# musheen/LevelSetFortran

Measured on AMD Instinct MI355X. Metric: cell-updates/s (WENO5 reinit, 512^3 fp64), higher is better.
Workload: dtype f64

## Files before the change

levelsetfortran_amd/csrc/lsf_cell.hpp:

```cpp
#pragma once
#include <hip/hip_runtime.h>

namespace lsf {

__device__ __forceinline__ double fmax2(double a, double b) { return (a > b) ? a : b; }
__device__ __forceinline__ double fmin2(double a, double b) { return (a < b) ? a : b; }
__device__ __forceinline__ double smax(double a, double b) { return __builtin_fmax(a, b); }
__device__ __forceinline__ double smin(double a, double b) { return __builtin_fmin(a, b); }

__device__ __forceinline__ double recip_refined(double d)
{
    double r = __builtin_amdgcn_rcp(d);
    double e = __builtin_fma(-d, r, 1.0);
    r = __builtin_fma(r, e, r);
    e = __builtin_fma(-d, r, 1.0);
    return __builtin_fma(r, e, r);
}
__device__ __forceinline__ double div_by(double n, double d, double r)
{
#pragma clang fp contract(off)
    const double q = n * r;
    const double e = __builtin_fma(-d, q, n);
    return __builtin_fma(e, r, q);
}
// ... 154 lines not shown
{
    double r = __builtin_amdgcn_rcp(x);
    const double e = __builtin_fma(-x, r, 1.0);
    return __builtin_fma(r, e, r);
}

__device__ __forceinline__ void weno_axis_fast(const double q[7], double floor2, bool yquirk, double& dm,
                                               double& dp)
{
    const double d0 = q[1] - q[0], d1 = q[2] - q[1], d2 = q[3] - q[2];
    const double d3 = q[4] - q[3], d4 = q[5] - q[4], d5 = q[6] - q[5];
    const double am = d1 - d0, bm = d2 - d1, cp = d3 - d2, bp = d4 - d3, ap = d5 - d4;
    const double e_ab = ap - bp, e_bc = bp - cp, e_cm = cp - bm, e_mm = am - bm;
    const double t0p = __builtin_fma(-3.0, bp, ap), t1p = bp + cp, t2p = __builtin_fma(3.0, cp, -bm);
    const double t0m = __builtin_fma(-3.0, bm, am), t1m = bm + cp, t2m = __builtin_fma(3.0, cp, -bp);

    const double mid = __builtin_fmax(__builtin_fmax(__builtin_fabs(d1), __builtin_fabs(d2)),
                                      __builtin_fmax(__builtin_fabs(d3), __builtin_fabs(d4)));
    const double mp = yquirk ? mid : __builtin_fmax(mid, __builtin_fabs(d5));
    const double mm = __builtin_fmax(mid, __builtin_fabs(d0));
    constexpr double C = 13.0 / 3.0;
    const double fl = C * floor2;
    const double epsp = __builtin_fma((1.E-6 / 3.0) * mp, mp, fl);
    const double epsm = __builtin_fma((1.E-6 / 3.0) * mm, mm, fl);

    const double c_ab = C * e_ab, c_bc = C * e_bc, c_cm = C * e_cm, c_mm = C * e_mm;
    const double q0p = __builtin_fma(t0p, t0p, __builtin_fma(c_ab, e_ab, epsp));
    const double q1p = __builtin_fma(t1p, t1p, __builtin_fma(c_bc, e_bc, epsp));
    const double q2p = __builtin_fma(t2p, t2p, __builtin_fma(c_cm, e_cm, epsp));
    const double q0m = __builtin_fma(t0m, t0m, __builtin_fma(c_mm, e_mm, epsm));
    const double q1m = __builtin_fma(t1m, t1m, __builtin_fma(c_cm, e_cm, epsm));
    const double q2m = __builtin_fma(t2m, t2m, __builtin_fma(c_bc, e_bc, epsm));

    const double S0 = e_bc - e_cm;
    const double S12 = S0 * (1.0 / 12.0), S0h = S0 * 0.5;
    const double t12p = q1p * q2p, t02p = q0p * q2p, t01p = q0p * q1p;
    const double t12m = q1m * q2m, t02m = q0m * q2m, t01m = q0m * q1m;
    const double n0p = t12p * t12p, n1p = t02p * t02p, m2p = t01p * t01p;
    const double n0m = t12m * t12m, n1m = t02m * t02m, m2m = t01m * t01m;
    const double Dp = __builtin_fma(3.0, m2p, __builtin_fma(6.0, n1p, n0p));
    const double Dm = __builtin_fma(3.0, m2m, __builtin_fma(6.0, n1m, n0m));
    const double R = rcp_nr(__builtin_fmax(Dp * Dm, 1e-300));
    const double rp = Dm * R, rm = Dp * R;
    const double Sap = e_ab - e_bc;
    const double Sam = e_mm + e_cm;
    const double PWp = __builtin_fma(rp, __builtin_fma(n0p * (1.0 / 3.0), Sap, m2p * S0h), -S12);
    const double PWm = __builtin_fma(rm, __builtin_fma(n0m * (1.0 / 3.0), Sam, m2m * S0h), -S12);
    const double cen12 = __builtin_fma(7.0, d2 + d3, -(d1 + d4));
    dm = __builtin_fma(1.0 / 12.0, cen12, -PWm);
    dp = __builtin_fma(1.0 / 12.0, cen12, PWp);
}

__device__ __forceinline__ void weno_iface_fast(const double v[6], double floor2, double& pwp, double& pwm, double& cen12)
{
#pragma clang fp contract(off)
    const double d1 = v[1] - v[0], d2 = v[2] - v[1], d3 = v[3] - v[2], d4 = v[4] - v[3], d5 = v[5] - v[4];
    const double um = d2 - d1, u0 = d3 - d2, u1 = d4 - d3, u2 = d5 - d4;
    const double e_ab = u2 - u1, e_bc = u1 - u0, e_cm = u0 - um;
    const double t0 = __builtin_fma(-3.0, u1, u2), t1 = u1 + u0, t2 = __builtin_fma(3.0, u0, -um);
    const double mx = __builtin_fmax(__builtin_fmax(__builtin_fmax(__builtin_fabs(d1), __builtin_fabs(d2)),
                                                    __builtin_fmax(__builtin_fabs(d3), __builtin_fabs(d4))),
                                     __builtin_fabs(d5));
    constexpr double C = 13.0 / 3.0;
    const double eps = __builtin_fma((1.E-6 / 3.0) * mx, mx, C * floor2);
    const double q0 = __builtin_fma(t0, t0, __builtin_fma(C * e_ab, e_ab, eps));
    const double q1 = __builtin_fma(t1, t1, __builtin_fma(C * e_bc, e_bc, eps));
    const double q2 = __builtin_fma(t2, t2, __builtin_fma(C * e_cm, e_cm, eps));
    const double t12 = q1 * q2, t02 = q0 * q2, t01 = q0 * q1;
    const double n0 = t12 * t12, n1 = t02 * t02, m2 = t01 * t01;
    const double Dp = __builtin_fma(3.0, m2, __builtin_fma(6.0, n1, n0));
    const double Dm = __builtin_fma(3.0, n0, __builtin_fma(6.0, n1, m2));
    const double R = rcp_nr(__builtin_fmax(Dp * Dm, 1e-300));
    const double rp = Dm * R, rm = Dp * R;
    const double Sa = e_ab - e_bc, S0 = e_bc - e_cm;
    const double A = n0 * Sa, B = m2 * S0;
    pwp = __builtin_fma(rp, __builtin_fma(A, 1.0 / 3.0, B * 0.5), -(S0 * (1.0 / 12.0)));
    pwm = __builtin_fma(rm, __builtin_fma(B, 1.0 / 3.0, A * 0.5), -(Sa * (1.0 / 12.0)));
    cen12 = __builtin_fma(7.0, d2 + d3, -(d1 + d4));
}

__device__ __forceinline__ void weno_axis_from_ifaces(const double q[7], double floor2, double& dm, double& dp)
{
#pragma clang fp contract(off)
    double pwp_l, pwm_c, cen_l, pwp_c, pwm_r, cen_c;
    weno_iface_fast(q, floor2, pwp_l, pwm_c, cen_l);
    weno_iface_fast(q + 1, floor2, pwp_c, pwm_r, cen_c);
    dm = __builtin_fma(1.0 / 12.0, cen_c, -pwm_c);
    dp = __builtin_fma(1.0 / 12.0, cen_c, pwp_c);
}


__device__ __forceinline__ double cell_update_fast(const double qx[7], const double qy[7],
                                                   const double qz[7], bool weno_ok, double pS, double dx,
                                                   double inv_dx, double floor2, double h)
{
    double a, b, c, d, e, f;
    if (weno_ok) {
        weno_axis_from_ifaces(qx, floor2, a, b);
        weno_axis_from_ifaces(qz, floor2, e, f);
    } else {
        a = qx[3] - qx[2], b = qx[4] - qx[3];
        e = qz[3] - qz[2], f = qz[4] - qz[3];
    }
    axis_pair<false>(qy, weno_ok, true, dx, floor2, c, d);
    const double phic = qx[3];
    return finish_update<false>(phic, axis_godunov<false>(phic, a, b), axis_godunov<false>(phic, c, d),
                                axis_godunov<false>(phic, e, f), pS, dx, inv_dx, h);
}

template <bool STRICT>
__device__ __forceinline__ double cell_update(const double qx[7], const double qy[7], const double qz[7],
                                              bool weno_ok, double pS, double dx, double inv_dx,
                                              double floor2, double h)
{
    if constexpr (STRICT)
        return cell_update_strict(qx, qy, qz, weno_ok, pS, dx, h);
    else
        return cell_update_fast(qx, qy, qz, weno_ok, pS, dx, inv_dx, floor2, h);
}

template <bool STRICT>
__device__ __forceinline__ void axis_pair(const double q[7], bool weno_ok, bool yquirk, double dx, double floor2,
                                          double& dm, double& dp)
{
    if constexpr (STRICT) {
#pragma clang fp contract(off)
        if (weno_ok) {
            weno_axis_strict(q, dx, yquirk, dm, dp);
        } else {
            const double rdx = recip_refined(dx);
            dm = div_dx(q[3] - q[2], dx, rdx);
            dp = div_dx(q[4] - q[3], dx, rdx);
        }
    } else {
        if (weno_ok) {
            weno_axis_fast(q, floor2, yquirk, dm, dp);
        } else {
            dm = q[3] - q[2];
            dp = q[4] - q[3];
        }
    }
}

template <bool STRICT>
__device__ __forceinline__ double axis_godunov(double phic, double dm, double dp)
{
#pragma clang fp contract(off)
    const double sg = phic > 0. ? 1.0 : -1.0;
    const double u = dm * sg, w = dp * -sg;
    const double m = STRICT ? smax(smax(u, w), 0.) : __builtin_fmax(__builtin_fmax(u, w), 0.);
    return m * m;
}

__device__ __forceinline__ double sqrt_unframed(double x)
{
#pragma clang fp contract(off)
    const double y = __builtin_amdgcn_rsq(x);
    double g = x * y, hh = y * 0.5;
    const double r = __builtin_fma(-hh, g, 0.5);
    g = __builtin_fma(g, r, g), hh = __builtin_fma(hh, r, hh);
    double d = __builtin_fma(-g, g, x);
    g = __builtin_fma(d, hh, g);
    d = __builtin_fma(-g, g, x);
    return __builtin_fma(d, hh, g);
}

__device__ __forceinline__ double rsqrt_nr(double t)
{
    const double y = __builtin_amdgcn_rsq(t);
    const double e = __builtin_fma(-0.5 * t * y, y, 0.5);
    return __builtin_fma(y, e, y);
}

template <bool STRICT>
__device__ __forceinline__ double finish_update(double phic, double gX, double gY, double gZ, double pS, double dx,
                                                double inv_dx, double h)
{
    if constexpr (STRICT) {
#pragma clang fp contract(off)
        const double S = gX + gY + gZ;
        const double pp = pS * pS, dd = dx * dx;
        if (__builtin_expect(S >= 1.0e-200 && S <= 1.0e200 && pp >= 1.0e-200 && pp <= 1.0e200 && dd >= 1.0e-200 && dd <= 1.0e200, 1)) {
            const double gM = sqrt_unframed(S);
            const double t = pp + dd * gM;
            const double den = sqrt_unframed(t);
            const double sgn = div_by(pS, den, recip_refined(den));
            const double k1 = sgn * (1. - gM);
            return phic + h * k1;
        }
        const double gM = __builtin_sqrt(S);
        const double sgn = pS / __builtin_sqrt(pS * pS + dx * dx * gM);
        const double k1 = sgn * (1. - gM);
        return phic + h * k1;
    } else {
        const double S = gX + gY + gZ;
        const double y0 = __builtin_amdgcn_rsq(__builtin_fmax(S, 1e-300));
        const double g0 = S * y0;
        const double g = __builtin_fma(__builtin_fma(-g0, g0, S), 0.5 * y0, g0);
        const double gM = g * inv_dx;
        const double sgn = pS * rsqrt_nr(__builtin_fma(pS, pS, dx * dx * gM));
        return __builtin_fma(h, sgn * (1. - gM), phic);
    }
}

__device__ __forceinline__ double minmax_curv(double c, double xp, double xm, double yp, double ym,
                                              double zp, double zm, double dxx)
{
#pragma clang fp contract(off)
    const double pxx = (-2. * c + xp + xm) * dxx;
    const double pyy = (-2. * c + yp + ym) * dxx;
    const double pzz = (-2. * c + zp + zm) * dxx;
    return pxx + pyy + pzz;
}

__device__ __forceinline__ double minmax_update(double c, double im, double ip, double jp, double jm,
                                                double kp, double km, double curv, double h1)
{
#pragma clang fp contract(off)
    double pAve = c + im + ip + jp + jm + kp + km;
    pAve = pAve / 7.;
    const double F = (pAve < 0.) ? fmin2(curv, 0.0) : fmax2(curv, 0.0);
    return c + h1 * F;
}

}
```

levelsetfortran_amd/csrc/lsf_skew.hpp:

```cpp
#pragma once
#include <hip/hip_runtime.h>
#include <stdint.h>

#include <type_traits>

#include "lsf_boxtile.hpp"

#ifndef LSF_SKEW_WIDE
#define LSF_SKEW_WIDE 1
#endif
#ifndef LSF_CELL_UNROLL
#define LSF_CELL_UNROLL 16
#endif

#ifndef LSF_STRICT22_WAVES
#define LSF_STRICT22_WAVES 4
#endif
#if !defined(LSF_EXPERIMENTS)
#undef LSF_PROBE_RA
#undef LSF_PROBE_RH
#endif
#ifndef LSF_PROBE_RA
#define LSF_PROBE_RA 0
#endif
// ... 128 lines not shown
struct SkShared {
    double lds[T::TOTAL];
    int2 rowtab[T::NR];
    double wsum[T::W];
};

template <class T>
__device__ __forceinline__ void sk_lane_offsets3(int axis, int si, int sj, int sk, bool deep, const SkPre& pre, int bc, int cc, int nj, int nk,
                                                 int (&off)[7])
{
    const bool pos = (axis == 0 ? si : (axis == 1 ? sj : sk)) > 0;
    if (deep) {
        const uint4 pk = pos ? pre.off1 : pre.off0;
        off[0] = (int)(pk.x & 0xffffu), off[1] = (int)(pk.x >> 16), off[2] = (int)(pk.y & 0xffffu), off[3] = (int)(pk.y >> 16);
        off[4] = (int)(pk.z & 0xffffu), off[5] = (int)(pk.z >> 16), off[6] = (int)(pk.w & 0xffffu);
    } else {
#pragma unroll
        for (int mm = 0; mm < 7; ++mm) off[mm] = T::lane_off(bc, cc, axis, pos, nj, nk, mm);
    }
#pragma unroll
    for (int mm = 0; mm < 7; ++mm) asm volatile("" : "+v"(off[mm]));
}
template <class T>
__device__ __forceinline__ void sk_lane_offsets1(int si, int sj, int sk, int bc, int cc, int nj, int nk, int (&ox)[7], int (&oy)[7], int (&oz)[7])
{
    constexpr int NYT = T::NYT, NZT = T::NZT;
    if (nj == NYT && nk == NZT) {
        constexpr int RA_ = T::RA, RH_ = T::RH, PS_ = NYT * T::RA + T::PAD;
        const int base = T::core_at(cc * NYT + bc) + 3;
        const int yu = T::HB + (T::YU0 - T::NCORE + cc * 3 + 3 + bc) * RH_ + 3, yd = T::HB + (T::YD0 - T::NCORE + cc * 3 + bc - NYT) * RH_ - 1;
        const int zu = T::HB + (T::ZU0 - T::NCORE + (cc + 3) * NYT + bc) * RH_ + 3, zd = T::HB + (T::ZD0 - T::NCORE + (cc - NZT) * NYT + bc) * RH_ - 1;
        int fy[7], fz[7];
#pragma unroll
        for (int d = -3; d <= 3; ++d) {
            const int bq = bc + d, cq = cc + d;
            fy[d + 3] = bq < 0 ? yu + d * (RH_ + 1) : (bq >= NYT ? yd + d * (RH_ + 1) : base + d * (RA_ + 1));
            fz[d + 3] = cq < 0 ? zu + d * (NYT * RH_ + 1) : (cq >= NZT ? zd + d * (NYT * RH_ + 1) : base + d * (PS_ + 1));
        }
#pragma unroll
        for (int mm = 0; mm < 7; ++mm) {
            ox[mm] = base + (si > 0 ? mm - 3 : 3 - mm);
            oy[mm] = sj > 0 ? fy[mm] : fy[6 - mm];
            oz[mm] = sk > 0 ? fz[mm] : fz[6 - mm];
        }
    } else {
#pragma unroll
        for (int mm = 0; mm < 7; ++mm) {
            ox[mm] = T::lane_off(bc, cc, 0, si > 0, nj, nk, mm);
            oy[mm] = T::lane_off(bc, cc, 1, sj > 0, nj, nk, mm);
            oz[mm] = T::lane_off(bc, cc, 2, sk > 0, nj, nk, mm);
        }
    }
#pragma unroll
    for (int mm = 0; mm < 7; ++mm) asm volatile("" : "+v"(ox[mm]), "+v"(oy[mm]), "+v"(oz[mm]));
}

#ifdef LSF_EXPERIMENTS
struct SkNoHook {
    __device__ __forceinline__ void operator()(int) const {}
};
#define LSF_SK_MID_TPARAM , class MidHook = SkNoHook
#define LSF_SK_MID_PARAM , MidHook mid = MidHook{}
#define LSF_SK_MID(t_) mid(t_)
#else
#define LSF_SK_MID_TPARAM
#define LSF_SK_MID_PARAM
#define LSF_SK_MID(t_)
#endif
template <int TA, int WY, int WZ, int BY, bool STRICT, bool SC1, bool PUSH = false, class WaitUp LSF_SK_MID_TPARAM>
__device__ __forceinline__ bool skew_tile(SkShared<SkTile<TA, WY, WZ, BY>>& sm, const GsArgs& a, uint32_t packed, int g, int si, int sj,
                                          int sk, const SkPre& pre, WaitUp&& wait_upstream LSF_SK_MID_PARAM)
{
    static_assert(TA == 16 || (TA == 32 && BY == 5 && !PUSH), "tiles of 32 marching steps: three lanes per cell, single launch only");
    constexpr int CPN = TA / 16;
    using T = SkTile<TA, WY, WZ, BY>;
    constexpr int NYT = T::NYT, NZT = T::NZT, W = T::W, NT = 64 * W;
    double* const lds = sm.lds;
    int2* const rowtab = sm.rowtab;
    double* const wsum = sm.wsum;
    int tid_ = threadIdx.x;
    if constexpr (PUSH) asm volatile("" : "+v"(tid_));
    const int tid = tid_, lane = tid & 63, wave = tid >> 6;
    const int nx = a.nx, ny = a.ny, nz = a.nz;
    const long sx = nx + 1, sxy = (long)(nx + 1) * (ny + 1);
    const double dx = a.dx, h = a.h;
    const double inv_dx = 1.0 / dx, floor2 = 1.E-99 * dx * dx / 13.0;
    const int ncol = a.nTj * a.nTk;

    constexpr bool SYS = PUSH;
    auto ldp = [](const double* p_) { return SYS ? ld_sys(p_) : (SC1 ? ld_sc1(p_) : *p_); };
    auto stp = [](double* p_, double v_) {
        if (SYS) st_sys(p_, v_);
        else if (SC1) st_sc1(p_, v_);
        else *p_ = v_;
    };

#ifdef LSF_EXPERIMENTS
    unsigned long long ph_[6];
#define LSF_PHASE(i_) ph_[i_] = __builtin_amdgcn_s_memrealtime()
#else
#define LSF_PHASE(i_)
#endif
    LSF_PHASE(0);
    const int m = packed & 0x3ff, fB = (packed >> 10) & 0x3ff, fC = (packed >> 20) & 0x3ff;
    const int tj = sj > 0 ? fB : a.nTj - 1 - fB, tk = sk > 0 ? fC : a.nTk - 1 - fC;
    const int j_lo = 1 + tj * NYT, k_lo = 1 + tk * NZT;
    const int nj = min(NYT, ny - j_lo), nk = min(NZT, nz - k_lo);
    const int nxi = nx - 1;
    const int X0 = TA * m - NYT * fB - NZT * fC;
    const int gb = a.nbuf == 4 ? (g & 3) : g % 3;
    const double* in = a.buf[gb];
    double* out = a.buf[gb + 1 == a.nbuf ? 0 : gb + 1];
    [[maybe_unused]] const int k_push_lo = PUSH ? 1 + a.tk_lo * NZT + 3 : 0, k_push_hi = PUSH ? min(1 + a.tk_hi * NZT, nz) - 3 : 0;
    [[maybe_unused]] double *nb_lo = nullptr, *nb_hi = nullptr;
    if constexpr (PUSH) {
        const int ob = gb + 1 == a.nbuf ? 0 : gb + 1;
        nb_lo = a.peers->nb_buf[0][ob], nb_hi = a.peers->nb_buf[1][ob];
    }

    const int org_j = max(j_lo - 3, 0), org_k = max(k_lo - 3, 0);
    const long org = sx * org_j + sxy * org_k;
    const double* in_t = in + org;
    double* out_t = out + org;
    const double* ps_t = a.phiS + org;
    const int gi0 = si > 0 ? 1 + X0 : nx - 1 - X0;
    const bool deep = a.tables && nj == NYT && nk == NZT && j_lo >= 4 && j_lo + NYT + 2 <= ny - 1 && k_lo >= 4 && k_lo + NZT + 2 <= nz - 1;
    const int dir = (sj > 0 ? 2 : 0) + (sk > 0 ? 1 : 0);
    for (int r = tid; r < T::NR; r += NT) {
        if (deep) {
            const uint32_t w = r == tid ? (dir == 0 ? pre.rel.x : (dir == 1 ? pre.rel.y : (dir == 2 ? pre.rel.z : pre.rel.w)))
                                        : a.tables[4 * r + dir];
            const int o = (int)(w & 63u) * (int)sx + (int)((w >> 6) & 63u) * (int)sxy, bc_ = (int)((w >> 12) & 255u) - 3;
            rowtab[r] = make_int2(o * 4 + (int)(w >> 20), si > 0 ? gi0 - bc_ : gi0 + bc_);
            continue;
        }
        int bq, cq, up, core;
        T::row_coords(r, nj, nk, &bq, &cq, &up, &core);
        const int gj_r = j_lo + (sj > 0 ? bq : nj - 1 - bq), gk_r = k_lo + (sk > 0 ? cq : nk - 1 - cq);
        const int rin = (int)((unsigned)(gj_r - 1) <= (unsigned)(ny - 2)) & (int)((unsigned)(gk_r - 1) <= (unsigned)(nz - 2));
        const int gj = min(max(gj_r, 0), ny), gk = min(max(gk_r, 0), nz);
        const int o = (gj - org_j) * (int)sx + (gk - org_k) * (int)sxy;
        rowtab[r] = make_int2(o * 4 + (rin & up) + 2 * (rin & (up | core)), si > 0 ? gi0 - (bq + cq) : gi0 + (bq + cq));
    }
    __syncthreads();
    LSF_PHASE(1);

    const int t16 = lane & 15;
    const int bl = BY == 5 ? t16 / 3 : t16, axis = BY == 5 ? t16 - 3 * bl : 0;
    const int b = BY * (wave % WY) + bl, c = 4 * (wave / WY) + (lane >> 4);
    const bool row_ok = bl < BY && b < nj && c < nk;
    const int bc = row_ok ? b : 0, cc = row_ok ? c : 0;
    constexpr int CU = LSF_CELL_UNROLL;
    static_assert(CU == 4 || CU == 8 || CU == 16, "steps per iteration of the one-lane-per-cell march");
    constexpr int NPS = BY == 5 ? TA / 2 : CU;
    double ps[NPS];
    double colsum_prev = 0.0;
    const int2 e_ps = rowtab[cc * NYT + bc];
    auto ps_load = [&](int t) {
        return ps_t[(unsigned)(e_ps.x >> 2) + (unsigned)min(max(e_ps.y + (si > 0 ? t : -t), 0), nx)];
    };
    const int gj = j_lo + (sj > 0 ? bc : nj - 1 - bc), gk = k_lo + (sk > 0 ? cc : nk - 1 - cc);
    const bool yz_weno = gj > 3 && gj < ny - 4 && gk > 3 && gk < nz - 4;
    const int fx0 = X0 - bc - cc;
    double acc = 0.0;
    auto step_mask = [](int lo_t, int hi_t) {
        lo_t = min(max(lo_t, 0), TA), hi_t = min(max(hi_t, lo_t), TA);
        return (unsigned)(((1ull << hi_t) - 1ull) & ~((1ull << lo_t) - 1ull));
    };
    const unsigned act_bits = row_ok ? step_mask(-fx0, nxi - fx0) : 0u;
    const unsigned weno_bits = yz_weno ? step_mask((si > 0 ? 3 : 4) - fx0, (si > 0 ? nx - 5 : nx - 4) - fx0) : 0u;

    [[maybe_unused]] bool yquirk = false;
    [[maybe_unused]] int row_core = 0;
    [[maybe_unused]] int off[7] = {0, 0, 0, 0, 0, 0, 0};
    [[maybe_unused]] int ox[7] = {0, 0, 0, 0, 0, 0, 0}, oy[7] = {0, 0, 0, 0, 0, 0, 0}, oz[7] = {0, 0, 0, 0, 0, 0, 0};
    if constexpr (BY == 5) {
        yquirk = axis == a.quirk_axis;
        row_core = T::core_at(cc * NYT + bc) + 3;
        sk_lane_offsets3<T>(axis, si, sj, sk, deep, pre, bc, cc, nj, nk, off);
    }
    typedef unsigned u4_t __attribute__((ext_vector_type(4)));
    constexpr int AUX_SC1 = SYS ? 17 : (SC1 ? 16 : 0);
    const bool widex = TA == 16 && (LSF_SKEW_WIDE == 2 || (LSF_SKEW_WIDE == 1 && BY == 16)) && deep && X0 - (NYT + NZT + 4) >= 0 && X0 + 22 <= nxi - 1 &&
                       sk_wide_image_fits(sxy, NZT);
    bool loaded = true;
    auto load_wide = [&]() {
        const __amdgpu_buffer_rsrc_t r_in = __builtin_amdgcn_make_buffer_rsrc(const_cast<double*>(in_t), 0, 0x7fffffff, 0x00020000);
        const __amdgpu_buffer_rsrc_t r_out = __builtin_amdgcn_make_buffer_rsrc(out_t, 0, 0x7fffffff, 0x00020000);
        constexpr int RPI = 4 * W;
        constexpr int NB = T::NCORE / RPI, NU = (T::YD0 - T::YU0 + RPI - 1) / RPI, ND = (T::NR - T::YD0 + RPI - 1) / RPI;
        constexpr int XC = 3 * T::NCORE, NXC = (XC + NT - 1) / NT;
        u4_t w[NB + ND + NU];
        int dw[NB + ND + NU];
        double v3[NXC + 1];
        int d3[NXC + 1];
        const int xx = tid & 15, rsub = tid >> 4;
        int n_ = 0;
        auto pair_at = [&](const __amdgpu_buffer_rsrc_t& rs, int2 e, int k) {
            const unsigned el = (unsigned)(e.x >> 2) + (unsigned)(e.y + (si > 0 ? k - 3 : 2 - k));
            return __builtin_amdgcn_raw_buffer_load_b128(rs, 8u * el, 0, AUX_SC1);
        };
#pragma unroll
        for (int u = 0; u < NB; ++u, ++n_) {
            const int r = RPI * u + rsub, k = 3 + 2 * min(xx, 9);
            dw[n_] = T::core_at(r) + k;
            w[n_] = pair_at(r_in, rowtab[r], k);
        }
#pragma unroll
        for (int u = 0; u < ND; ++u, ++n_) {
            const int r = min(T::YD0 + RPI * u + rsub, T::NR - 1), k = 4 + 2 * min(xx, 8);
            dw[n_] = T::HB + (r - T::NCORE) * T::RH + k - 4;
            w[n_] = pair_at(r_in, rowtab[r], k);
        }
#pragma unroll
        for (int t = 0; t < NPS; ++t) ps[t] = ps_load(t);
        if constexpr (BY == 16) sk_lane_offsets1<T>(si, sj, sk, bc, cc, nj, nk, ox, oy, oz);
        if (!wait_upstream()) {
            loaded = false;
            return;
        }
        if (tid == 0 && m != (NYT * fB + NZT * fC) / TA) colsum_prev = ldp(a.colsum + (long)gb * ncol + (tj + (long)a.nTj * tk));
#pragma unroll
        for (int u = 0; u < NU; ++u, ++n_) {
            const int r = min(T::YU0 + RPI * u + rsub, T::YD0 - 1), k = 2 * min(xx, 8);
            dw[n_] = T::HB + (r - T::NCORE) * T::RH + k;
            w[n_] = pair_at(r_out, rowtab[r], k);
        }
#pragma unroll
        for (int u = 0; u < NXC; ++u) {
            const int idx = min(tid + NT * u, XC - 1);
            const int r = idx / 3, k = idx - 3 * r;
            const int2 e = rowtab[r];
            d3[u] = T::core_at(r) + k;
            v3[u] = ldp((const double*)out_t + ((unsigned)(e.x >> 2) + (unsigned)(e.y + (si > 0 ? k - 3 : 3 - k))));
        }
#pragma unroll
        for (int u = 0; u < NB + ND + NU; ++u) {
            const double lo = __hiloint2double((int)w[u].y, (int)w[u].x), hi = __hiloint2double((int)w[u].w, (int)w[u].z);
            lds[dw[u]] = si > 0 ? lo : hi;
            if (u >= NB || xx < 9) lds[dw[u] + 1] = si > 0 ? hi : lo;
        }
#pragma unroll
        for (int u = 0; u < NXC; ++u) lds[d3[u]] = v3[u];
    };
    auto load_rows = [&]() {
        constexpr int RPI = 4 * W;
        constexpr int NB = T::NCORE / RPI * CPN;
        constexpr int NU = (T::YD0 - T::YU0 + RPI - 1) / RPI * CPN;
        constexpr int ND = (T::NR - T::YD0 + RPI - 1) / RPI * CPN;
        constexpr int XC = 3 * T::NCORE, XHU = 2 * (T::YD0 - T::NCORE), XHD = 2 * (T::NR - T::YD0);
        constexpr int NXC = (XC + NT - 1) / NT, NXHU = (XHU + NT - 1) / NT, NXHD = (XHD + NT - 1) / NT;
        constexpr int NV = NB + NU + ND + 2 * NXC + NXHU + NXHD;
        double v[NV];
        int dst[NV];
        const int xx = tid & 15, rsub = tid >> 4;
        int n_ = 0;
        auto gi_of = [&](int2 e, int k) { return e.y + (si > 0 ? k - 3 : 3 - k); };
        auto off_of = [&](int2 e, int gi_r) { return (unsigned)(e.x >> 2) + (unsigned)min(max(gi_r, 0), nx); };
#pragma unroll
        for (int u = 0; u < NB; ++u, ++n_) {
            const int r = RPI * (u / CPN) + rsub, k = 3 + xx + 16 * (u % CPN);
            const int2 e = rowtab[r];
            dst[n_] = T::core_at(r) + k;
            v[n_] = ldp(in_t + off_of(e, gi_of(e, k)));
        }
#pragma unroll
        for (int u = 0; u < ND; ++u, ++n_) {
            const int r = min(T::YD0 + RPI * (u / CPN) + rsub, T::NR - 1), k = 4 + xx + 16 * (u % CPN);
            const int2 e = rowtab[r];
            dst[n_] = T::HB + (r - T::NCORE) * T::RH + k - 4;
            v[n_] = ldp(in_t + off_of(e, gi_of(e, k)));
        }
#pragma unroll
        for (int u = 0; u < NXC; ++u, ++n_) {
            const int idx = min(tid + NT * u, XC - 1);
            const int r = idx / 3, k = TA + 3 + idx - 3 * r;
            const int2 e = rowtab[r];
            dst[n_] = T::core_at(r) + k;
            v[n_] = ldp(in_t + off_of(e, gi_of(e, k)));
        }
#pragma unroll
        for (int u = 0; u < NXHD; ++u, ++n_) {
            const int hh = min(tid + NT * u, XHD - 1);
            const int r = T::YD0 + (hh >> 1), k = TA + 4 + (hh & 1);
            const int2 e = rowtab[r];
            dst[n_] = T::at(r, k);
            v[n_] = ldp(in_t + off_of(e, gi_of(e, k)));
        }
#pragma unroll
        for (int t = 0; t < NPS; ++t) ps[t] = ps_load(t);
        if constexpr (BY == 16) sk_lane_offsets1<T>(si, sj, sk, bc, cc, nj, nk, ox, oy, oz);
        if (!wait_upstream()) {
            loaded = false;
            return;
        }
        if (tid == 0 && m != (NYT * fB + NZT * fC) / TA) colsum_prev = ldp(a.colsum + (long)gb * ncol + (tj + (long)a.nTj * tk));
#pragma unroll
        for (int u = 0; u < NU; ++u, ++n_) {
            const int r = min(T::YU0 + RPI * (u / CPN) + rsub, T::YD0 - 1), k = 2 + xx + 16 * (u % CPN);
            const int2 e = rowtab[r];
            const int gi_r = gi_of(e, k);
            const bool fresh = ((unsigned)(gi_r - 1) <= (unsigned)(nx - 2)) & (bool)(e.x & 1);
            dst[n_] = T::HB + (r - T::NCORE) * T::RH + k;
            v[n_] = ldp((fresh ? (const double*)out_t : in_t) + off_of(e, gi_r));
        }
#pragma unroll
        for (int u = 0; u < NXC; ++u, ++n_) {
            const int idx = min(tid + NT * u, XC - 1);
            const int r = idx / 3, k = idx - 3 * r;
            const int2 e = rowtab[r];
            const int gi_r = gi_of(e, k);
            const bool fresh = ((unsigned)(gi_r - 1) <= (unsigned)(nx - 2)) & (bool)(e.x & 2);
            dst[n_] = T::core_at(r) + k;
            v[n_] = ldp((fresh ? (const double*)out_t : in_t) + off_of(e, gi_r));
        }
#pragma unroll
        for (int u = 0; u < NXHU; ++u, ++n_) {
            const int hh = min(tid + NT * u, XHU - 1);
            const int r = T::NCORE + (hh >> 1), k = hh & 1;
            const int2 e = rowtab[r];
            const int gi_r = gi_of(e, k);
            const bool fresh = ((unsigned)(gi_r - 1) <= (unsigned)(nx - 2)) & (bool)(e.x & 2);
            dst[n_] = T::at(r, k);
            v[n_] = ldp((fresh ? (const double*)out_t : in_t) + off_of(e, gi_r));
        }
#pragma unroll
        for (int u = 0; u < NV; ++u) lds[dst[u]] = v[u];
    };
    if (widex) load_wide();
    else load_rows();
    if (!loaded) return false;
    __syncthreads();
    LSF_PHASE(2);

    if constexpr (BY == 5) {
        {
#pragma unroll
            for (int t = 0; t < TA; ++t) {
                LSF_SK_MID(t);
                const bool active = (bool)((act_bits >> t) & 1u) && axis == 0;
                double q[7];
#pragma unroll
                for (int mm = 0; mm < 7; ++mm) q[mm] = lds[off[mm] + t];
                const double pS = ps[t & (TA / 2 - 1)];
                if (t + TA / 2 < TA) ps[t & (TA / 2 - 1)] = ps_load(t + TA / 2);
                const bool weno_ok = (bool)((weno_bits >> t) & 1u);
                double dm, dp;
                axis_pair<STRICT>(q, weno_ok, yquirk, dx, floor2, dm, dp);
                const double gg = axis_godunov<STRICT>(q[3], dm, dp);
                const double gX = gg, gY = dpp_mov<0x101>(gg), gZ = dpp_mov<0x102>(gg);
                if (active) {
                    const double newv = finish_update<STRICT>(q[3], gX, gY, gZ, pS, dx, inv_dx, h);
                    lds[row_core + t] = newv;
                    const double dlt = newv - q[3];
                    acc = STRICT ? acc + dlt * dlt : __builtin_fma(dlt, dlt, acc);
                }
                __syncthreads();
            }
        }
    } else {
        const bool quirk_x = a.quirk_axis == 0, quirk_y = a.quirk_axis == 1;
#pragma unroll 1
        for (int t0 = 0; t0 < TA; t0 += CU) {
#pragma unroll
            for (int u = 0; u < CU; ++u) {
                const int t = t0 + u;
                LSF_SK_MID(t);
                const bool active = (act_bits >> t) & 1u;
                const bool weno_ok = (weno_bits >> t) & 1u;
                double qx[7], qy[7], qz[7];
#pragma unroll
                for (int mm = 0; mm < 7; ++mm) qx[mm] = lds[ox[mm] + t];
#pragma unroll
                for (int mm = 0; mm < 7; ++mm) qy[mm] = mm == 3 ? qx[3] : lds[oy[mm] + t];
#pragma unroll
                for (int mm = 0; mm < 7; ++mm) qz[mm] = mm == 3 ? qx[3] : lds[oz[mm] + t];
                const double pS = ps[u];
                if (STRICT ? CU < TA : (CU < TA && t0 + CU < TA)) ps[u] = ps_load(min(t + CU, TA - 1));
                if (active) {
                    const double c0 = qx[3];
                    double xm, xp, ym, yp, zm, zp;
                    axis_pair<STRICT>(qx, weno_ok, quirk_x, dx, floor2, xm, xp);
                    axis_pair<STRICT>(qy, weno_ok, quirk_y, dx, floor2, ym, yp);
                    axis_pair<STRICT>(qz, weno_ok, false, dx, floor2, zm, zp);
                    const double newv = finish_update<STRICT>(c0, axis_godunov<STRICT>(c0, xm, xp), axis_godunov<STRICT>(c0, ym, yp),
                                                              axis_godunov<STRICT>(c0, zm, zp), pS, dx, inv_dx, h);
                    lds[ox[3] + t] = newv;
                    const double dlt = newv - c0;
                    acc = STRICT ? acc + dlt * dlt : __builtin_fma(dlt, dlt, acc);
                }
                if (W > 1) asm volatile("s_waitcnt lgkmcnt(0)\n\ts_barrier" ::: "memory");
            }
        }
    }

    LSF_PHASE(3);
    const int fx_min = X0 - (nj - 1) - (nk - 1), fx_max = X0 + TA - 1;
    const bool near_wall = j_lo == 1 || j_lo + nj == ny || k_lo == 1 || k_lo + nk == nz ||
                           (fx_min <= 0 && fx_max >= 0) || (fx_min <= nxi - 1 && fx_max >= nxi - 1);
    if (widex) {
        const __amdgpu_buffer_rsrc_t r_out = __builtin_amdgcn_make_buffer_rsrc(out_t, 0, 0x7fffffff, 0x00020000);
        __builtin_amdgcn_s_waitcnt(0x0F70);
#pragma unroll
        for (int u = 0; u < (T::NCORE + 8 * W - 1) / (8 * W); ++u) {
            const int r = 8 * W * u + (tid >> 3), t = 2 * (tid & 7);
            if (r < T::NCORE) {
                const int2 e = rowtab[r];
                const double v0 = lds[T::core_at(r) + 3 + t], v1 = lds[T::core_at(r) + 4 + t];
                const double lo = si > 0 ? v0 : v1, hi = si > 0 ? v1 : v0;
                u4_t pk;
                pk.x = (unsigned)__double2loint(lo), pk.y = (unsigned)__double2hiint(lo);
                pk.z = (unsigned)__double2loint(hi), pk.w = (unsigned)__double2hiint(hi);
                const unsigned el = (unsigned)(e.x >> 2) + (unsigned)(e.y + (si > 0 ? t : -t - 1));
                __builtin_amdgcn_raw_buffer_store_b128(pk, r_out, 8u * el, 0, AUX_SC1);
                if constexpr (PUSH) {
                    const int cq = r / NYT, gk2 = k_lo + (sk > 0 ? cq : nk - 1 - cq);
                    if (nb_lo && gk2 < k_push_lo)
                        __builtin_amdgcn_raw_buffer_store_b128(pk, __builtin_amdgcn_make_buffer_rsrc(nb_lo + org, 0, 0x7fffffff, 0x00020000), 8u * el, 0, AUX_SC1);
                    if (nb_hi && gk2 >= k_push_hi)
                        __builtin_amdgcn_raw_buffer_store_b128(pk, __builtin_amdgcn_make_buffer_rsrc(nb_hi + org, 0, 0x7fffffff, 0x00020000), 8u * el, 0, AUX_SC1);
                }
            }
        }
    } else {
    constexpr int NUW = T::NCORE / (4 * W) * CPN;
#ifndef LSF_WB_CHUNK
#define LSF_WB_CHUNK 3
#endif
#ifndef LSF_WB_CHUNK16
#define LSF_WB_CHUNK16 3
#endif
    constexpr int GWC = BY == 16 ? LSF_WB_CHUNK16 : LSF_WB_CHUNK;
    constexpr int GW = NUW < GWC ? NUW : GWC;
    struct WbRow {
        int cq, t, gi, gj2, gk2, ai, aj, ak;
        int2 e;
        bool mine;
    };
    auto wb_row_e = [&](int u, int2 e_) {
        WbRow w;
        const int r = 4 * W * (u / CPN) + (tid >> 4);
        w.cq = r / NYT;
        const int bq = r - NYT * w.cq;
        w.t = (tid & 15) + 16 * (u % CPN);
        w.e = e_;
        w.gi = w.e.y + (si > 0 ? w.t : -w.t);
        w.mine = bq < nj && w.cq < nk && (unsigned)(w.gi - 1) <= (unsigned)(nx - 2);
        w.gj2 = j_lo + (sj > 0 ? bq : nj - 1 - bq), w.gk2 = k_lo + (sk > 0 ? w.cq : nk - 1 - w.cq);
        w.ai = w.gi == 1 ? -1 : (w.gi == nx - 1 ? 1 : 0), w.aj = w.gj2 == 1 ? -1 : (w.gj2 == ny - 1 ? 1 : 0);
        w.ak = w.gk2 == 1 ? -1 : (w.gk2 == nz - 1 ? 1 : 0);
        return w;
    };
    auto wb_row = [&](int u) { return wb_row_e(u, rowtab[4 * W * (u / CPN) + (tid >> 4)]); };
    auto sub_on = [](const WbRow& w, int sub) { return !(((sub & 1) && !w.ai) || ((sub & 2) && !w.aj) || ((sub & 4) && !w.ak)); };
    if (near_wall) {
#pragma unroll
        for (int u0 = 0; u0 < NUW; u0 += GW) {
            double oldw[GW][7];
            bool any = false;
#pragma unroll
            for (int g_ = 0; g_ < GW; ++g_) {
                if (u0 + g_ >= NUW) break;
                const WbRow w = wb_row(u0 + g_);
                any = any || (w.mine && (w.ai | w.aj | w.ak));
#pragma unroll
                for (int sub = 1; sub < 8; ++sub) {
                    oldw[g_][sub - 1] = 0.0;
                    if (!w.mine || !sub_on(w, sub)) continue;
                    const int wi = w.gi + ((sub & 1) ? w.ai : 0), wj = w.gj2 + ((sub & 2) ? w.aj : 0), wk = w.gk2 + ((sub & 4) ? w.ak : 0);
                    oldw[g_][sub - 1] = ldp(in + (wi + sx * wj + sxy * wk));
                }
            }
            if (__builtin_amdgcn_ballot_w64(any) == 0ull) continue;
#pragma unroll
            for (int g_ = 0; g_ < GW; ++g_) {
                const int u = u0 + g_;
                if (u >= NUW) break;
                const WbRow w = wb_row(u);
                if (!(w.mine && (w.ai | w.aj | w.ak))) continue;
                const double val0 = lds[T::core_at(4 * W * (u / CPN) + (tid >> 4)) + 3 + w.t];
#pragma unroll
                for (int sub = 1; sub < 8; ++sub) {
                    if (!sub_on(w, sub)) continue;
                    const int wi = w.gi + ((sub & 1) ? w.ai : 0), wj = w.gj2 + ((sub & 2) ? w.aj : 0), wk = w.gk2 + ((sub & 4) ? w.ak : 0);
                    const int nb = __builtin_popcount(sub);
                    const int nh = (int)(wi == nx) + (int)(wj == ny) + (int)(wk == nz);
                    const int mrep = min(nb, 1 + nh);
                    double val = val0;
                    {
#pragma clang fp contract(off)
                        for (int rr = 0; rr < mrep; ++rr) val = val + dx;
                    }
                    const long p = wi + sx * wj + sxy * wk;
                    const double dlt = val - oldw[g_][sub - 1];
                    stp(out + p, val);
                    if constexpr (PUSH) {
                        if (nb_lo && wk < k_push_lo) st_sys(nb_lo + p, val);
                        if (nb_hi && wk >= k_push_hi) st_sys(nb_hi + p, val);
                    }
                    acc = STRICT ? acc + dlt * dlt : __builtin_fma(dlt, dlt, acc);
                }
            }
// ... 3 lines not shown
    int2 e_wb[NUW];
    double v_wb[NUW];
#pragma unroll
    for (int u = 0; u < NUW; ++u) {
        e_wb[u] = rowtab[4 * W * (u / CPN) + (tid >> 4)];
        v_wb[u] = lds[T::core_at(4 * W * (u / CPN) + (tid >> 4)) + 3 + (tid & 15) + 16 * (u % CPN)];
    }
#pragma unroll
    for (int u = 0; u < NUW; ++u) asm volatile("" : "+v"(e_wb[u].x), "+v"(e_wb[u].y), "+v"(v_wb[u]));
#pragma unroll
    for (int u = 0; u < NUW; ++u) {
        const WbRow w = wb_row_e(u, e_wb[u]);
        const double val0 = v_wb[u];
        if (w.mine) stp(out_t + ((unsigned)(w.e.x >> 2) + (unsigned)w.gi), val0);
        if constexpr (PUSH) {
            if (w.mine && nb_lo && w.gk2 < k_push_lo) st_sys(nb_lo + org + ((unsigned)(w.e.x >> 2) + (unsigned)w.gi), val0);
            if (w.mine && nb_hi && w.gk2 >= k_push_hi) st_sys(nb_hi + org + ((unsigned)(w.e.x >> 2) + (unsigned)w.gi), val0);
        }
    }
    }
    acc = wave_sum_x(acc);
    if (W > 1) {
        if (lane == 0) wsum[wave] = acc;
        __syncthreads();
        acc = wsum[0];
        for (int w = 1; w < W; ++w) acc += wsum[w];
    }

    if (tid == 0) {
        double* slot = a.colsum + (long)gb * ncol + (tj + (long)a.nTj * tk);
        stp(slot, colsum_prev + acc);
        if constexpr (PUSH) {
            const int epi = sk > 0 ? a.nslab - 1 : 0;
            if (epi != a.slab) st_sys(a.peers->all_colsum[epi] + (long)gb * ncol + (tj + (long)a.nTj * tk), colsum_prev + acc);
        }
    }
    if (SC1) asm volatile("s_waitcnt vmcnt(0)" ::: "memory");
#ifdef LSF_EXPERIMENTS
    if (a.dbg) {
        asm volatile("s_waitcnt vmcnt(0)" ::: "memory");
        LSF_PHASE(4);
        if (tid == 0) {
            for (int i_ = 0; i_ < 4; ++i_) atomicAdd(a.dbg + 3 + i_, ph_[i_ + 1] - ph_[i_]);
            atomicAdd(a.dbg + 7, 1ull);
        }
    }
#endif
    if (packed != a.last_packed) return true;
    __syncthreads();
    if (wave != 0) return true;
    const double* cs = a.colsum + (long)gb * ncol;
    double tsum = 0.0;
    for (int p = lane; p < ncol; p += 64) tsum += ldp(cs + p);
    tsum = wave_sum(tsum);
    if (lane == 0) {
        const double rms = __builtin_sqrt(tsum / a.den);
        if constexpr (PUSH) {
            const bool stop = rms < a.tol || rms != rms || ld_flag_sys(a.ctl + 0) != 0;
            const SlabPeers* pe = a.peers;
            for (int q = 0; q < a.nslab; ++q) {
                if (g < a.trace_cap) st_sys(pe->all_trace[q] + g, rms);
                st_flag_sys(pe->all_ctl[q] + 1, g + 1);
                if (rms != rms) st_flag_sys(pe->all_ctl[q] + 2, 1);
                if (stop) st_flag_sys(pe->all_ctl[q] + 0, 1);
                st_flag_sys(pe->all_verdict[q] + (g - a.g0), stop ? 2 : 1);
            }
        } else {
            if (g < a.trace_cap) a.trace[g] = rms;
            st_flag(a.ctl + 1, g + 1);
            if (rms < a.tol) st_flag(a.ctl + 0, 1);
            else if (rms != rms) { st_flag(a.ctl + 2, 1); st_flag(a.ctl + 0, 1); }
        }
    }
    return true;
}

static __global__ __launch_bounds__(256) void k_transpose_xy(const double* __restrict__ src, double* __restrict__ dst, int ex, int ey,
                                                      long planes, double* __restrict__ dst2)
{
    __shared__ double t[32][33];
    const int tx = threadIdx.x & 31, ty = threadIdx.x >> 5;
    const int i0 = blockIdx.x * 32, j0 = blockIdx.y * 32;
    const long pl = (long)ex * ey;
    for (long k = blockIdx.z; k < planes; k += gridDim.z) {
        const double* s = src + k * pl;
        double* d = dst + k * pl;
#pragma unroll
        for (int r = 0; r < 4; ++r) {
            const int j = j0 + ty + 8 * r, i = i0 + tx;
            if (i < ex && j < ey) t[ty + 8 * r][tx] = s[i + (long)ex * j];
        }
        __syncthreads();
#pragma unroll
        for (int r = 0; r < 4; ++r) {
            const int i = i0 + ty + 8 * r, j = j0 + tx;
            if (i < ex && j < ey) {
                const double v = t[tx][ty + 8 * r];
                d[j + (long)ey * i] = v;
                if (dst2) dst2[k * pl + j + (long)ey * i] = v;
            }
        }
        __syncthreads();
    }
}

static __global__ __launch_bounds__(256) void k_build_order(uint2* __restrict__ order, const uint32_t* __restrict__ tiles,
                                                     const int* __restrict__ plane_off, const int* __restrict__ start,
                                                     const unsigned* __restrict__ slot_base, int ns, int np)
{
    const int slot = blockIdx.x;
    unsigned base = slot_base[slot];
    for (int q = 0; q < ns; ++q) {
        const int P = slot - start[q];
        if (P < 0) break;
        if (P >= np) continue;
        const int o = plane_off[P], cnt = plane_off[P + 1] - o;
        const unsigned tag = (unsigned)q | ((unsigned)P << DF_SWEEP_BITS);
        for (int i = threadIdx.x; i < cnt; i += 256) order[base + i] = make_uint2(tiles[o + i], tag);
        base += (unsigned)cnt;
    }
}

template <int TA, int WY, int WZ, int BY, bool STRICT>
__global__ __launch_bounds__(64 * WY * WZ) __attribute__((amdgpu_waves_per_eu(BY == 16 ? (WY * WZ == 1 ? 1 : LSF_WAVES16) : (WY == 2 && WZ == 2 ? (TA == 32 ? 2 : 5) : 1)))) void k_reinit_gs_skew(GsArgs a)
{
    const int bx = (int)blockIdx.x;
    const int seg = (bx >= a.seg_end[0]) + (bx >= a.seg_end[1]) + (bx >= a.seg_end[2]);
    const uint32_t packed = a.seg_tiles[seg][bx - (seg ? a.seg_end[seg - 1] : 0)];
    if (ld_flag(a.ctl + 0) != 0) return;
#ifdef LSF_EXPERIMENTS
    if (a.ticket && a.probe_us > 0) {
        if (threadIdx.x == 0) {
            const unsigned hw = __builtin_amdgcn_s_getreg((31 << 11) | 4), xcc = __builtin_amdgcn_s_getreg((31 << 11) | 20);
            const int ord = atomicAdd(a.ticket + ((xcc & 7u) * 256u + ((hw >> 8) & 255u)), 1);
            if (ord == 1) {
                const unsigned long long t0 = __builtin_amdgcn_s_memrealtime();
                while (__builtin_amdgcn_s_memrealtime() - t0 < 100ull * (unsigned)a.probe_us) __builtin_amdgcn_s_sleep(32);
            }
        }
        __syncthreads();
    }
#endif
#if defined(LSF_EXPERIMENTS) && defined(LSF_PROBE_LDS_PAD)
    __shared__ int lds_pad[LSF_PROBE_LDS_PAD / 4];
    if (a.nx < 0) lds_pad[threadIdx.x] = a.ny, a.ctl[5] = lds_pad[threadIdx.x ^ 1];
#endif
    const SkPre pre = sk_prefetch<TA, WY, WZ, BY>(a);
    __shared__ SkShared<SkTile<TA, WY, WZ, BY>> sm;
    skew_tile<TA, WY, WZ, BY, STRICT, false>(sm, a, packed, a.seg_g[seg], a.seg_sign[seg][0], a.seg_sign[seg][1], a.seg_sign[seg][2], pre,
                                             [] { return true; });
}

template <int TA, int WY, int WZ, int BY, bool STRICT>
__global__ __launch_bounds__(64 * WY * WZ) __attribute__((amdgpu_waves_per_eu(BY == 16 ? (WY * WZ == 1 ? 1 : LSF_WAVES16) : (WY == 2 && WZ == 2 ? (TA == 32 ? 2 : (STRICT ? LSF_STRICT22_WAVES : 5)) : 1)))) void k_reinit_gs_persist(GsArgs a)
{
    using T = SkTile<TA, WY, WZ, BY>;
    __shared__ SkShared<T> sm;
    __shared__ int sh_task[8];
    const int tid = threadIdx.x;
    const int np = a.np;
    const int nM = a.nM;
    const long per_sweep = (long)nM * a.nTj * a.nTk;
    {
        const unsigned long long tsA = a.dbg ? __builtin_amdgcn_s_memrealtime() : 0ull;
        const SkPre pre = sk_prefetch<TA, WY, WZ, BY>(a);
        const int* const set_word = a.ctl + 4;
        const int *w0 = set_word, *w1 = set_word, *w2 = set_word;
        unsigned long long t0 = 0;
        bool up_ready = false;
        auto give_up = [&]() {
            __hip_atomic_fetch_max(a.ticket, (int)a.total, __ATOMIC_RELAXED, __HIP_MEMORY_SCOPE_AGENT);
        };
        if (tid == 0) {
            const long t = (long)__hip_atomic_fetch_add(a.ticket, 1, __ATOMIC_RELAXED, __HIP_MEMORY_SCOPE_AGENT);
            int go = 0;
            uint2 e = make_uint2(0u, 0u);
            if (t < a.total) {
                e = a.order[t];
                const int s = (int)(e.y & (unsigned)(DF_BATCH - 1)), P = (int)(e.y >> DF_SWEEP_BITS);
                const int m = e.x & 0x3ff, B = (e.x >> 10) & 0x3ff, C = (e.x >> 20) & 0x3ff;
                auto m_lo = [&](int B_, int C_) { return (T::NYT * B_ + T::NZT * C_) / TA; };
                auto m_hi = [&](int B_, int C_) { return (T::NYT * B_ + T::NYT - 1 + T::NZT * C_ + T::NZT - 1 + a.nx - 2) / TA; };
                const int* td = a.tile_done + s * per_sweep;
                w0 = m - 1 >= m_lo(B, C) ? td + (m - 1) + (long)nM * (B + (long)a.nTj * C) : set_word;
                w1 = (B >= 1 && m >= m_lo(B - 1, C) && m <= m_hi(B - 1, C)) ? td + m + (long)nM * (B - 1 + (long)a.nTj * C) : set_word;
                w2 = (C >= 1 && m >= m_lo(B, C - 1) && m <= m_hi(B, C - 1)) ? td + m + (long)nM * (B + (long)a.nTj * (C - 1)) : set_word;
                const int* pd = a.planes_done;
                const int4 swp = *(const int4*)(a.sweep_tab + 4 * s);
                const int need3 = s < a.nbuf ? 0 : np + 1;
                const int* always = a.ctl + 1;
                const int* p3 = s == 0 ? always : pd + s - 1;
                const int* p4 = s < a.nbuf ? always : pd + s - a.nbuf;
                t0 = __builtin_amdgcn_s_memrealtime();
                go = 1;
                for (;;) {
                    const int vstop = ld_flag(a.ctl + 0);
                    const int v3 = ld_flag(p3), v4 = ld_flag(p4);
                    const int u0 = ld_flag(w0), u1 = ld_flag(w1), u2 = ld_flag(w2);
                    up_ready = (u0 != 0) & (u1 != 0) & (u2 != 0);
                    int h = swp.w;
                    asm volatile("" : "+v"(h));
                    const int need1 = s == 0 ? 0 : min(P + h, np);
                    if (vstop != 0) {
                        go = 2;
                        give_up();
                        break;
                    }
                    if ((v3 >= need1) & (v4 >= need3)) {
                        if (s >= a.nbuf && v4 == np + 2) {
                            go = 2;
                            give_up();
                        }
                        break;
                    }
                    if (__builtin_amdgcn_s_memrealtime() - t0 > a.timeout_ticks) {
                        st_flag(a.ctl + 2, 2);
                        st_flag(a.ctl + 0, 1);
                        go = 2;
                        break;
                    }
                    __builtin_amdgcn_s_sleep(LSF_POLL_SLEEP);
                }
                sh_task[3] = swp.x, sh_task[4] = swp.y, sh_task[5] = swp.z;
            }
            sh_task[0] = (int)e.x, sh_task[1] = (int)e.y, sh_task[2] = go, sh_task[7] = up_ready ? 1 : 0;
        }
        __syncthreads();
        auto uni = [](int v) { return __builtin_amdgcn_readfirstlane(v); };
        const uint32_t packed = (uint32_t)uni(sh_task[0]);
        const int sP = uni(sh_task[1]);
        int go = uni(sh_task[2]);
        const bool upstream_done = uni(sh_task[7]) != 0;
        const int s = sP & (DF_BATCH - 1), P = (int)((unsigned)sP >> DF_SWEEP_BITS);
        if (go == 0) return;
        typedef __attribute__((address_space(1))) int* GlobalIntPtr;
        GlobalIntPtr my_flag;
        {
            const int m_ = packed & 0x3ff, B_ = (packed >> 10) & 0x3ff, C_ = (packed >> 20) & 0x3ff;
            my_flag = (GlobalIntPtr)(a.tile_done + s * per_sweep + m_ + (long)nM * (B_ + (long)a.nTj * C_));
            asm volatile("" : "+s"(my_flag));
        }
        const unsigned long long tsB = a.dbg ? __builtin_amdgcn_s_memrealtime() : 0ull;
        auto wait_upstream = [&]() -> bool {
            if (upstream_done) return true;
            if (tid == 0) {
                int go2 = 1;
                for (;;) {
                    const int vstop = ld_flag(a.ctl + 0);
                    const int v0 = ld_flag(w0), v1 = ld_flag(w1), v2 = ld_flag(w2);
                    if (vstop != 0) {
                        go2 = 2;
                        give_up();
                        break;
                    }
                    if ((v0 != 0) & (v1 != 0) & (v2 != 0)) break;
                    if (__builtin_amdgcn_s_memrealtime() - t0 > a.timeout_ticks) {
                        st_flag(a.ctl + 2, 2);
                        st_flag(a.ctl + 0, 1);
                        go2 = 2;
                        break;
                    }
                    __builtin_amdgcn_s_sleep(LSF_POLL_SLEEP);
                }
                sh_task[6] = go2;
            }
            asm volatile("s_waitcnt lgkmcnt(0)\n\ts_barrier" ::: "memory");
            return uni(sh_task[6]) == 1;
        };
        if (go == 1) {
#ifdef LSF_EXPERIMENTS
            auto early = [&](int t) {
                if (a.probe_early > 0 && t == a.probe_early && tid == 0) __hip_atomic_store(my_flag, 1, __ATOMIC_RELAXED, LSF_FLAG_ST_SCOPE);
            };
            if (!skew_tile<TA, WY, WZ, BY, STRICT, true>(sm, a, packed, a.g0 + s, uni(sh_task[3]), uni(sh_task[4]), uni(sh_task[5]), pre, wait_upstream, early))
                go = 2;
#else
            if (!skew_tile<TA, WY, WZ, BY, STRICT, true>(sm, a, packed, a.g0 + s, uni(sh_task[3]), uni(sh_task[4]), uni(sh_task[5]), pre, wait_upstream))
                go = 2;
#endif
            asm volatile("s_waitcnt vmcnt(0)" ::: "memory");
        }
        __syncthreads();
        if (tid == 0 && go == 1) {
            __hip_atomic_store(my_flag, 1, __ATOMIC_RELAXED, LSF_FLAG_ST_SCOPE);
            const int done = __hip_atomic_fetch_add(a.plane_cnt + s * np + P, 1, __ATOMIC_RELAXED, __HIP_MEMORY_SCOPE_AGENT) + 1;
            if (done == a.plane_size[P]) {
                for (;;) {
                    int lead = ld_flag(a.planes_done + s);
                    if (lead >= np || ld_flag(a.plane_cnt + s * np + lead) < a.plane_size[lead]) break;
                    int next = lead + 1;
                    if (next == np) next = np + 1 + (ld_flag(a.ctl + 0) != 0 ? 1 : 0);
                    __hip_atomic_compare_exchange_strong(a.planes_done + s, &lead, next, __ATOMIC_RELAXED, __ATOMIC_RELAXED,
                                                         __HIP_MEMORY_SCOPE_AGENT);
                }
            }
            if (a.dbg) {
                const unsigned long long tsC = __builtin_amdgcn_s_memrealtime();
                atomicAdd(a.dbg + 0, tsB - tsA);
                atomicAdd(a.dbg + 1, tsC - tsB);
                atomicAdd(a.dbg + 2, 1ull);
            }
        }
    }
}

static __global__ __launch_bounds__(256) void k_build_order_slab(uint2* __restrict__ order, const uint32_t* __restrict__ tiles_pos,
                                                          const uint32_t* __restrict__ tiles_neg, const int* __restrict__ off_pos,
// ... 170 lines not shown
```

Measured before the change: 51.46 billion.

## Split sign-source loads across axis lanes, specialise Godunov branch, cap waves

In the BY==5 path, each of the three axis lanes now preloads one third of the sign/source values. Values held by other lanes are fetched with DPP moves instead of a rolling per-step reload, which cuts per-lane register and load pressure. The Godunov term is rewritten as a select between two precomputed maxima and wrapped in an axis_term helper that branches on weno_ok, with an asm barrier on the fallback path. An upper waves-per-EU bound is added for the strict 2x2 TA=16 kernel. The risks are extra cross-lane DPP traffic, code size from the branch split, and possible lane-mapping errors in the ps redistribution.

```diff
diff --git a/levelsetfortran_amd/csrc/lsf_cell.hpp b/levelsetfortran_amd/csrc/lsf_cell.hpp
--- a/levelsetfortran_amd/csrc/lsf_cell.hpp
+++ b/levelsetfortran_amd/csrc/lsf_cell.hpp
@@ -330,6 +330,31 @@
     return m * m;
 }
 
+template <bool STRICT>
+__device__ __forceinline__ double axis_godunov_sel(double phic, double dm, double dp)
+{
+#pragma clang fp contract(off)
+    const double mpos = STRICT ? smax(dm, -dp) : __builtin_fmax(dm, -dp);
+    const double mneg = STRICT ? smax(-dm, dp) : __builtin_fmax(-dm, dp);
+    const double mo = phic > 0. ? mpos : mneg;
+    const double m = STRICT ? smax(mo, 0.) : __builtin_fmax(mo, 0.);
+    return m * m;
+}
+
+template <bool STRICT>
+__device__ __forceinline__ double axis_term(const double q[7], bool weno_ok, bool yquirk, double dx, double floor2)
+{
+    double dm, dp;
+    if (weno_ok) {
+        axis_pair<STRICT>(q, true, yquirk, dx, floor2, dm, dp);
+        return axis_godunov_sel<STRICT>(q[3], dm, dp);
+    }
+    axis_pair<STRICT>(q, false, yquirk, dx, floor2, dm, dp);
+    double g = axis_godunov_sel<STRICT>(q[3], dm, dp);
+    asm volatile("" : "+v"(g));
+    return g;
+}
+
 __device__ __forceinline__ double sqrt_unframed(double x)
 {
 #pragma clang fp contract(off)
diff --git a/levelsetfortran_amd/csrc/lsf_skew.hpp b/levelsetfortran_amd/csrc/lsf_skew.hpp
--- a/levelsetfortran_amd/csrc/lsf_skew.hpp
+++ b/levelsetfortran_amd/csrc/lsf_skew.hpp
@@ -304,12 +304,14 @@
     const int bc = row_ok ? b : 0, cc = row_ok ? c : 0;
     constexpr int CU = LSF_CELL_UNROLL;
     static_assert(CU == 4 || CU == 8 || CU == 16, "steps per iteration of the one-lane-per-cell march");
-    constexpr int NPS = BY == 5 ? TA / 2 : CU;
+    constexpr int NPS = BY == 5 ? (TA + 2) / 3 : CU;
     double ps[NPS];
     double colsum_prev = 0.0;
     const int2 e_ps = rowtab[cc * NYT + bc];
+    const int ps_t0 = BY == 5 ? NPS * axis : 0;
+    const int ps_gi0 = e_ps.y + (si > 0 ? ps_t0 : -ps_t0);
     auto ps_load = [&](int t) {
-        return ps_t[(unsigned)(e_ps.x >> 2) + (unsigned)min(max(e_ps.y + (si > 0 ? t : -t), 0), nx)];
+        return ps_t[(unsigned)(e_ps.x >> 2) + (unsigned)min(max(ps_gi0 + (si > 0 ? t : -t), 0), nx)];
     };
     const int gj = j_lo + (sj > 0 ? bc : nj - 1 - bc), gk = k_lo + (sk > 0 ? cc : nk - 1 - cc);
     const bool yz_weno = gj > 3 && gj < ny - 4 && gk > 3 && gk < nz - 4;
@@ -494,12 +496,9 @@
                 double q[7];
 #pragma unroll
                 for (int mm = 0; mm < 7; ++mm) q[mm] = lds[off[mm] + t];
-                const double pS = ps[t & (TA / 2 - 1)];
-                if (t + TA / 2 < TA) ps[t & (TA / 2 - 1)] = ps_load(t + TA / 2);
+                const double pS = t < NPS ? ps[t] : (t < 2 * NPS ? dpp_mov<0x101>(ps[t - NPS]) : dpp_mov<0x102>(ps[t - 2 * NPS]));
                 const bool weno_ok = (bool)((weno_bits >> t) & 1u);
-                double dm, dp;
-                axis_pair<STRICT>(q, weno_ok, yquirk, dx, floor2, dm, dp);
-                const double gg = axis_godunov<STRICT>(q[3], dm, dp);
+                const double gg = axis_term<STRICT>(q, weno_ok, yquirk, dx, floor2);
                 const double gX = gg, gY = dpp_mov<0x101>(gg), gZ = dpp_mov<0x102>(gg);
                 if (active) {
                     const double newv = finish_update<STRICT>(q[3], gX, gY, gZ, pS, dx, inv_dx, h);
@@ -809,7 +808,7 @@
 }
 
 template <int TA, int WY, int WZ, int BY, bool STRICT>
-__global__ __launch_bounds__(64 * WY * WZ) __attribute__((amdgpu_waves_per_eu(BY == 16 ? (WY * WZ == 1 ? 1 : LSF_WAVES16) : (WY == 2 && WZ == 2 ? (TA == 32 ? 2 : (STRICT ? LSF_STRICT22_WAVES : 5)) : 1)))) void k_reinit_gs_persist(GsArgs a)
+__global__ __launch_bounds__(64 * WY * WZ) __attribute__((amdgpu_waves_per_eu(BY == 16 ? (WY * WZ == 1 ? 1 : LSF_WAVES16) : (WY == 2 && WZ == 2 ? (TA == 32 ? 2 : (STRICT ? LSF_STRICT22_WAVES : 5)) : 1), (BY == 5 && WY == 2 && WZ == 2 && TA == 16 && STRICT) ? LSF_STRICT22_WAVES : 8))) void k_reinit_gs_persist(GsArgs a)
 {
     using T = SkTile<TA, WY, WZ, BY>;
     __shared__ SkShared<T> sm;
```

Result: faster. 53.06 billion (median of 6 runs) (+3.1%).
